# projectchrono/DEM-Engine

Hardware: AMD Instinct MI355X
Metric: clump*steps/s (higher is better)
Workload: dtype f32 physics / f64 geometry

## Files before the change

### dem-engine_amd/abi.py

```python
import ctypes as C
import os

import numpy as np

_HERE = os.path.dirname(os.path.abspath(__file__))

NULL_MAPPING_PARTNER = 0xFFFFFFFF
FAMILY_MASK_ENTRIES = 32896
NUM_FAMILIES = 256
FAMILY_FIXED = 1
FAMILY_GHOST = 2
FAMILY_PRESCRIBED = 4
INTEGRATOR_FORWARD_EULER, INTEGRATOR_CENTERED_DIFFERENCE, INTEGRATOR_EXTENDED_TAYLOR = 0, 1, 2
FORCE_HERTZIAN, FORCE_HERTZIAN_FRICTIONLESS, FORCE_CUSTOM = 0, 1, 2
GHOST_BYTES = 56


ARITH_FAST, ARITH_EXACT = 1, 0


class DemeParams(C.Structure):
    _fields_ = [
        ("nvXp2", C.c_uint32), ("nvYp2", C.c_uint32), ("nvZp2", C.c_uint32),
        ("nbX", C.c_uint32), ("nbY", C.c_uint32), ("nbZ", C.c_uint32),
# ... 145 lines not shown
        "deme_integrate": [_P], "deme_step": [_P, C.c_uint32],
        "deme_get_counts": [_P, C.POINTER(DemeCounts)],
        "deme_download_bin_incidence": [_P, _P, _P, C.c_size_t],
        "deme_download_contacts": [_P, _P, _P, _P, _P, C.c_size_t],
        "deme_download_contact_wildcard": [_P, C.c_uint32, _P, C.c_size_t],
        "deme_upload_contact_wildcard": [_P, C.c_uint32, _P, C.c_size_t],
        "deme_seed_contacts": [_P, _P, _P, _P, _P, C.c_size_t],
        "deme_compile_prescriptions": [_P, C.c_char_p, C.c_char_p, C.c_char_p],
        "deme_upload_wildcard_array": [_P, C.c_uint32, C.c_uint32, _P, C.c_size_t],
        "deme_download_wildcard_array": [_P, C.c_uint32, C.c_uint32, _P, C.c_size_t],
        "deme_halo_stream": [_P, C.POINTER(_P)], "deme_halo_pack_async": [_P, _P, C.c_uint32, _P],
        "deme_halo_unpack_async": [_P, _P, C.c_uint32, _P], "deme_halo_sync": [_P],
        "deme_step_overlap_begin": [_P, C.POINTER(C.c_int)], "deme_step_overlap_end": [_P],
        "deme_compile_family_rules": [_P, C.c_char_p], "deme_change_family": [_P, C.c_uint32, C.c_uint32],
        "deme_set_family_material": [_P, C.c_uint32, C.c_uint32, C.c_int],
        "deme_device_memory": [_P, C.POINTER(C.c_size_t), C.POINTER(C.c_size_t)],
        "deme_set_adaptive": [_P, C.POINTER(DemeAdaptive)],
        "deme_get_adaptive_state": [_P, C.POINTER(C.c_double), C.POINTER(C.c_uint32), C.POINTER(C.c_uint32), C.POINTER(C.c_uint32)],
        "deme_mark_persistent_contacts": [_P, C.c_int, C.c_uint32, C.c_uint32, C.c_int],
        "deme_num_persistent_contacts": [_P, C.POINTER(C.c_size_t)],
        "deme_add_owner_acc": [_P, C.c_uint32, C.c_uint32, _P, _P],
        "deme_download_persistent_contacts": [_P, _P, _P, _P, C.c_size_t],
        "deme_upload_persistent_contacts": [_P, _P, _P, _P, C.c_size_t],
        "deme_inspect": [_P, C.c_uint32, C.POINTER(C.c_float)],
        "deme_compile_region": [_P, C.c_char_p, C.POINTER(C.c_int)],
        "deme_inspect_region": [_P, C.c_uint32, C.c_int, C.POINTER(C.c_float)],
        "deme_upload_volumes": [_P, _P, C.c_size_t], "deme_inspect_values": [_P, C.c_uint32, _P, C.c_size_t],
        "deme_set_record_contacts": [_P, C.c_int],
        "deme_download_contact_records": [_P, _P, _P, _P, _P, C.c_size_t],
        "deme_download_sphere_geometry": [_P, _P, _P, _P, _P, C.c_size_t],
        "deme_query_owner_contacts": [_P, _P, C.c_size_t, C.c_int, _P, _P, _P, _P, _P, _P, _P, _P, _P, _P, C.c_size_t,
                                      C.POINTER(C.c_size_t)],
        "deme_query_host_bytes": [_P, C.POINTER(C.c_uint64)],
        "deme_change_owner_sizes": [_P, _P, _P, C.c_size_t], "deme_num_components": [_P, C.POINTER(C.c_uint32)],
        "deme_download_components": [_P, _P, _P, _P, _P, C.c_size_t], "deme_download_sphere_components": [_P, _P, C.c_size_t],
        "deme_set_template_components": [_P, C.c_uint32], "deme_multi_change_owner_sizes": [_P, _P, _P, C.c_size_t],
        "deme_multi_download_sphere_components": [_P, _P, C.c_size_t],
        "deme_compile_force_model": [_P, C.c_char_p, C.c_size_t, C.POINTER(C.c_char_p), C.c_uint32, C.c_char_p],
        "deme_compile_force_model_ex": [_P, C.c_char_p, C.c_size_t, C.POINTER(C.c_char_p), C.c_uint32, C.POINTER(C.c_char_p),
                                        C.c_uint32, C.POINTER(C.c_char_p), C.c_uint32, C.c_char_p],
        "deme_kernel_time_ms": [_P, C.c_char_p, C.POINTER(C.c_double), C.POINTER(C.c_uint64)],
        "deme_kernel_time_reset": [_P], "deme_set_timing": [_P, C.c_int],
        "deme_halo_pack": [_P, _P, C.c_uint32, _P], "deme_halo_unpack": [_P, _P, C.c_uint32, _P],
        "deme_jit_probe": [C.c_char_p, C.POINTER(C.c_char_p), C.c_uint32, C.c_char_p, C.c_char_p, C.c_size_t],
        "deme_jit_probe_ex": [C.c_char_p, C.POINTER(C.c_char_p), C.c_uint32, C.POINTER(C.c_char_p), C.c_uint32,
                              C.POINTER(C.c_char_p), C.c_uint32, C.c_char_p, C.c_char_p, C.c_size_t],
    }.items():
        fn = getattr(lib, name)
        fn.argtypes = args
        fn.restype = C.c_int
    lib.deme_halo_unique_id.argtypes = [_P]
    lib.deme_halo_unique_id.restype = C.c_int
    lib.deme_halo_group_create.argtypes = [_P, C.c_int, C.c_int, C.c_int, C.POINTER(_P)]
    lib.deme_halo_group_create.restype = C.c_int
    lib.deme_halo_group_destroy.argtypes = [_P]
    lib.deme_halo_group_destroy.restype = None
    lib.deme_halo_group_last_error.argtypes = [_P]
    lib.deme_halo_group_last_error.restype = C.c_char_p
    lib.deme_halo_group_attach.argtypes = [_P, _P, C.c_int, _P, _P, C.c_uint32, _P, C.c_uint32, C.c_int, _P, _P, C.c_uint32, _P, C.c_uint32]
    lib.deme_halo_group_attach.restype = C.c_int
    for name, args in {"deme_halo_group_step": [_P, C.c_uint32], "deme_halo_group_exchange": [_P], "deme_halo_group_sync": [_P],
                       "deme_halo_group_stats": [_P, C.POINTER(C.c_uint64), C.POINTER(C.c_uint64)]}.items():
        getattr(lib, name).argtypes = args
        getattr(lib, name).restype = C.c_int
    _lib = lib
    return lib


def halo_unique_id():
    buf = (C.c_ubyte * 128)()
    if load_library().deme_halo_unique_id(buf) != 0:
        raise DemeError("RCCL is not available (deme_halo_unique_id)")
    return bytes(buf)


class HaloGroup:

    def __init__(self, rank=0, world=1, device=0, unique_id=None):
        self.lib = load_library()
        h = _P()
        idbuf = None if unique_id is None else (C.c_ubyte * 128).from_buffer_copy(unique_id)
        rc = self.lib.deme_halo_group_create(idbuf, int(rank), int(world), int(device), C.byref(h))
        self.h = h
# ... 358 lines not shown
        self._ck(self.lib.deme_multi_download_contact_wildcard(self.h, int(w), _ptr(out), n), "deme_multi_download_contact_wildcard")
        return out

    def contact_records(self):
        n = self.num_contacts()
        arrs = [np.zeros((n, 3), np.float32) for _ in range(4)]
        self.lib.deme_multi_download_contact_records.argtypes = [_P, _P, _P, _P, _P, C.c_size_t]
        self._ck(self.lib.deme_multi_download_contact_records(self.h, *[_ptr(a) for a in arrs], n), "deme_multi_download_contact_records")
        return arrs

    def close(self):
        if getattr(self, "h", None):
            self.lib.deme_multi_destroy(self.h)
            self.h = None

    def __del__(self):
        try:
            self.close()
        except Exception:
            pass


def exported_symbols():
    import re
    hdr = os.path.join(_HERE, "..", "include", "deme_hip.h")
    txt = open(hdr).read()
    return sorted(set(re.findall(r"\b(deme_[a-z_0-9]+)\s*\(", txt)))


def _ptr(a):
    return None if a is None else a.ctypes.data


def jit_probe(src, wildcard_names=(), prerequisites="", owner_wildcards=(), geo_wildcards=()):
    lib = load_library()

    def arr(ns):
        return (C.c_char_p * max(1, len(ns)))(*[s.encode() for s in ns])
    log = C.create_string_buffer(8192)
    rc = lib.deme_jit_probe_ex(src.encode(), arr(wildcard_names), len(wildcard_names), arr(owner_wildcards), len(owner_wildcards),
                               arr(geo_wildcards), len(geo_wildcards), prerequisites.encode(), log, len(log))
    return rc == 0, log.value.decode(errors="replace")


class Context:

    def __init__(self, device=0):
        self.lib = load_library()
        h = _P()
        rc = self.lib.deme_ctx_create(int(device), C.byref(h))
        if rc != 0 or not h:
            raise DemeError(f"deme_ctx_create failed (status {rc}): is a HIP device visible?")
        self.h = h
        self.n_owners = 0
        self.n_spheres = 0
        self.n_wildcards = 0

    @classmethod
    def borrowed(cls, handle):
        self = cls.__new__(cls)
        self.lib = load_library()
        self.h = handle
        self._borrowed = True
        v = (C.c_uint32 * 4)()
        self.lib.deme_scene_sizes.argtypes = [_P, C.POINTER(C.c_uint32)]
        self._ck(self.lib.deme_scene_sizes(self.h, v), "deme_scene_sizes")
# ... 377 lines not shown
```

### dem-engine_amd/csrc/deme_hip.hip

```cpp
#include <algorithm>
#include <cmath>
#include <cstdarg>
#include <cstdio>
#include <cstdlib>
#include <chrono>
#include <cstring>
#include <condition_variable>
#include <functional>
#include <memory>
#include <mutex>
#include <dlfcn.h>
#include <map>
#include <string>
#include <thread>
#include <vector>

#include <hip/hip_runtime.h>
#include <rocprim/rocprim.hpp>
template <unsigned RB, unsigned IPT = 8>
using DemeRadixCfg = rocprim::radix_sort_config<rocprim::default_config, rocprim::default_config,
                                                rocprim::radix_sort_onesweep_config<rocprim::kernel_config<1024, IPT>, rocprim::kernel_config<1024, IPT>, RB,
                                                                                    rocprim::block_radix_rank_algorithm::match>,
                                                1024 * 1024>;
#include <array>
#include <iterator>
#include <limits>

#include "../../include/deme_hip.h"
#include "deme_device.h"
#include "deme_force.h"
#include "deme_force_fast.h"
#include "deme_jit.h"
#include "deme_kernels.h"
#include "deme_tile.h"
#include "deme_tile_step.h"
#include "deme_migrate.h"
#include "deme_mesh_kernels.h"
#include "deme_resize.h"
#include "deme_query.h"

using namespace deme_dev;

namespace {

struct DevBuf {
    void* p = nullptr;
    size_t bytes = 0;
    template <typename T>
    T* as() const {
        return reinterpret_cast<T*>(p);
    }
};

struct ContactList {
    DevBuf mapping, ownerA, ownerB[2], bIdx[2], info, tInfo, rIdx, lPos, remVal, rankC, remKey[2], cDefer, blockMode, smFlag, smList;
    DevBuf aStart, bStart, heavy, fixedFlag, heavyList, rangeCtr, hList, hCount, tileMode, tileOrg, rStart, lOff, lCount, tileRem, tileBase,
        tileBig, bigList;
    uint64_t nListed = 0;
    int listKeys = 0;
    bool legacyLists = false;
    bool tileActive = false;
    bool fusedList = false;
    bool fusedChecked = false;
    bool hrPending = false, heavyOverflow = false;
    uint32_t nHeavy = 0, nHeavyFree = 0, nSA = 0, nSM = 0;
    uint32_t nBigTiles = 0, tileMaxHalo = 0, tileMaxList = 0, tileMaxHaloIn = 0;

    void invalidate() {
        nListed = 0, listKeys = 0;
        legacyLists = tileActive = fusedList = fusedChecked = hrPending = heavyOverflow = false;
        nHeavy = nHeavyFree = nSA = nSM = 0;
        nBigTiles = tileMaxHalo = tileMaxList = tileMaxHaloIn = 0;
// ... 193 lines not shown
        HIPCK(hipMemcpyAsync(np, b.p, b.bytes, hipMemcpyDeviceToDevice, c->stream));
    if (b.p) {
        HIPCK(hipStreamSynchronize(c->stream));
        HIPCK(hipFree(b.p));
    }
    b.p = np;
    b.bytes = want;
    return DEME_OK;
}

template <typename T>
int upload(deme_ctx* c, DevBuf& b, const T* src, size_t n) {
    int rc = ensure(c, b, std::max<size_t>(n, 1) * sizeof(T));
    if (rc)
        return rc;
    if (n && src)
        HIPCK(hipMemcpyAsync(b.p, src, n * sizeof(T), hipMemcpyHostToDevice, c->stream));
    else if (n)
        HIPCK(hipMemsetAsync(b.p, 0, n * sizeof(T), c->stream));
    return DEME_OK;
}

template <class Call>
int with_temp(deme_ctx* c, DevBuf& tmp, Call&& call) {
    size_t bytes = 0;
    HIPCK(call(nullptr, bytes));
    if (int rc = ensure(c, tmp, bytes))
        return rc;
    bytes = tmp.bytes;
    HIPCK(call(tmp.p, bytes));
    return DEME_OK;
}

inline unsigned grid_for(size_t n, unsigned block = 256) { return (unsigned)((n + block - 1) / block); }
inline unsigned bits_for(uint64_t n, unsigned cap) {
    unsigned b = 1;
    while (b < cap && (1ull << b) < n)
        b++;
    return b;
}

hipEvent_t get_event(deme_ctx* c) {
    if (!c->eventPool.empty()) {
        hipEvent_t e = c->eventPool.back();
        c->eventPool.pop_back();
        return e;
    }
    hipEvent_t e;
    hipEventCreate(&e);
    return e;
}
struct ScopedTimer {
    deme_ctx* c;
    TimerSlot* slot = nullptr;
    hipEvent_t a = nullptr, b = nullptr;
    hipStream_t st = nullptr;
    ScopedTimer(deme_ctx* ctx, const char* name, bool always = false, hipStream_t stream = nullptr) : c(ctx), st(stream ? stream : ctx->stream) {
        if (!c->timing)
            return;
        slot = &c->timers[name];
        if (!always && (slot->seen++ % (uint64_t)c->timing) != 0) {
            slot = nullptr;
            return;
        }
        if (slot->pending.size() >= 8192) {
            slot = nullptr;
// ... 235 lines not shown
                return fail(c, DEME_ERR_OVERFLOW,
                            "a sphere touches more than %u bins (margin far larger than the bin size): the incidence list cannot be built",
                            DEME_MAX_BINS_PER_SPHERE);
            if ((uint64_t)hc.maxCount * nS > 0xFFFFFFFFull) {
                auto in64 = rocprim::make_transform_iterator(c->counts.as<uint32_t>(),
                                                             [] __host__ __device__(uint32_t v) { return (unsigned long long)v; });
                unsigned long long* tot = &c->ctr.as<DetectCounters>()->nContactsRaw;
                unsigned long long keep = 0, total = 0;
                HIPCK(hipMemcpyAsync(&keep, tot, 8, hipMemcpyDeviceToHost, st));
                if (int rc = with_temp(c, c->sortTmp, [&](void* tmp, size_t& bytes) {
                        return rocprim::reduce(tmp, bytes, in64, tot, 0ull, (size_t)nS, rocprim::plus<unsigned long long>(), st);
                    }))
                    return rc;
                HIPCK(hipMemcpyAsync(&total, tot, 8, hipMemcpyDeviceToHost, st));
                HIPCK(hipStreamSynchronize(st));
                HIPCK(hipMemcpyAsync(tot, &keep, 8, hipMemcpyHostToDevice, st));
                HIPCK(hipStreamSynchronize(st));
                if (total > 0xFFFFFFFFull)
                    return fail(c, DEME_ERR_OVERFLOW, "%llu bin-sphere incidences do not fit the 32-bit list offsets (use larger bins)", total);
            }
        }
        if (P > c->incCap) {
            if (int rc = grow_incidence_arena(c, (size_t)P + P / 4 + 1024))
                return rc;
            filled = false;
        }
        c->nInc = P;
        const unsigned bits = bits_for((uint64_t)c->hp.nbX * c->hp.nbY * c->hp.nbZ, 32);
        if (P) {
            if (!filled)
                fill_incidence();
            const bool twoPass = bits > 16 && bits <= 22;
            if (int rc = with_temp(c, c->sortTmp, [&](void* tmp, size_t& bytes) {
                    return twoPass ? rocprim::radix_sort_pairs<DemeRadixCfg<11, 16>>(tmp, bytes, c->incKeys[0].as<uint32_t>(), c->incKeys[1].as<uint32_t>(),
                                                                                     c->incVals[0].as<uint32_t>(), c->incVals[1].as<uint32_t>(), (size_t)P, 0, bits, st)
                                   : rocprim::radix_sort_pairs<DemeRadixCfg<8>>(tmp, bytes, c->incKeys[0].as<uint32_t>(), c->incKeys[1].as<uint32_t>(),
                                                                                c->incVals[0].as<uint32_t>(), c->incVals[1].as<uint32_t>(), (size_t)P, 0, bits, st);
                }))
                return rc;
            const uint32_t nWin = (uint32_t)grid_for(P, SW_T);
            if (int rc = ensure(c, c->binStat, (size_t)nWin * sizeof(uint2)))
                return rc;
            static_assert(SW_WPB == 1, "k_sweep writes one statistics record per window");
            hipLaunchKernelGGL(k_sweep, dim3(nWin), dim3(SW_T), 0, st, c->dp,
                               c->incKeys[1].as<uint32_t>(), c->incVals[1].as<uint32_t>(), P, c->geo.as<GeoRec>(),
                               c->sphFam.as<uint16_t>(), ar, c->binStat.as<uint2>());
            hipLaunchKernelGGL(k_bin_stats_final, dim3((nWin + 2047u) / 2048u), dim3(256), 0, st, c->binStat.as<uint2>(), nWin,
                               c->ctr.as<DetectCounters>());
        }
        c->nTriInc = 0;
        if (c->nTri && P) {
            const uint32_t nT = c->nTri;
            hipLaunchKernelGGL(k_tri_prep, dim3(grid_for(nT)), dim3(256), 0, st, c->dp, nT, c->tris.as<TriRec>(),
                               ow, c->triWorld.as<TriWorld>(), c->triLo.as<int4>(),
                               c->triHi.as<int4>(), c->triCounts.as<uint32_t>());
            size_t tmp = c->scanTmp.bytes;
            HIPCK(rocprim::exclusive_scan(c->scanTmp.p, tmp, c->triCounts.as<uint32_t>(), c->triOffsets.as<uint32_t>(), 0u,
                                          (size_t)nT + 1, rocprim::plus<uint32_t>(), st));
            uint32_t TP = 0;
            HIPCK(hipMemcpyAsync(&TP, c->triOffsets.as<uint32_t>() + nT, 4, hipMemcpyDeviceToHost, st));
            HIPCK(hipStreamSynchronize(st));
            if (TP > c->triCap) {
                const size_t cap = (size_t)TP + TP / 4 + 1024;
                for (int k = 0; k < 2; k++)
                    if (ensure(c, c->triKeys[k], cap * 4) || ensure(c, c->triVals[k], cap * 4))
                        return c->lastStatus;
                c->triCap = cap;
            }
            c->nTriInc = TP;
            if (TP) {
// ... 53 lines not shown
                        "a bin contains %u sphere components, exceeding the allowance %u (SetMaxSphereInBin)", c->maxInBin,
                        c->dp.errOutBinSphNum);
        uint64_t nC = hc.nContactsRaw;
        const size_t nPersist = c->hPersist.size();
        if (nPersist) {
            if (nC + nPersist > c->cntCap) {
                if (async)
                HIPCK(hipStreamSynchronize(c->stream));
            if (int rc = grow_contact_arena(c, (size_t)nC + nPersist + nC / 4 + 1024))
                    return rc;
                continue;
            }
            nC += nPersist;
        }
        const int next = c->keysCur ^ 1;
        uint64_t* rawKeys = c->keysRaw.as<uint64_t>();
        if (segmented) {
            c->lastSegMax = segMax;
            if (grid_for(segMax) > compactBlocks)
                hipLaunchKernelGGL(k_compact_keys, dim3((unsigned)grid_for(segMax) - compactBlocks, DEME_KEY_SEGS), dim3(256), 0, st,
                                   c->keysRaw.as<uint64_t>(), ar.segCap, c->segCtr.as<unsigned long long>(), compactBlocks,
                                   c->keysSorted[next].as<uint64_t>());
            if (hc.nContactsRaw)
                rawKeys = c->keysSorted[next].as<uint64_t>();
        }
        if (nPersist)
            HIPCK(hipMemcpyAsync(rawKeys + hc.nContactsRaw, c->persistKeys.p, nPersist * 8, hipMemcpyDeviceToDevice, st));
        if (nC) {
            const unsigned bitsA = bits_for(c->dp.nSpheres, 31);
            if (int rc = ensure(c, c->keysMid, (size_t)c->cntCap * 8))
                return rc;
            uint64_t* mid = c->keysMid.as<uint64_t>();
            if (int rc = with_temp(c, c->sortTmp, [&](void* tmp, size_t& bytes) {
                    return rocprim::radix_sort_keys<DemeRadixCfg<8>>(tmp, bytes, rawKeys, mid, (size_t)nC, 31, 33 + bitsA, st);
                }))
                return rc;
            hipLaunchKernelGGL(k_segment_rank_sort, dim3(grid_for(nC)), dim3(256), 0, st, (uint32_t)nC, mid,
                               c->keysSorted[next].as<uint64_t>());
            if (nPersist) {
                unsigned long long* cnt = &c->ctr.as<DetectCounters>()->nContactsRaw;
                if (int rc = with_temp(c, c->scanTmp, [&](void* tmp, size_t& bytes) {
                        return rocprim::unique(tmp, bytes, c->keysSorted[next].as<uint64_t>(), c->keysRaw.as<uint64_t>(), cnt, (size_t)nC,
                                               rocprim::equal_to<uint64_t>(), st);
                    }))
                    return rc;
                unsigned long long nU = 0;
                HIPCK(hipMemcpyAsync(&nU, cnt, 8, hipMemcpyDeviceToHost, st));
                HIPCK(hipStreamSynchronize(st));
                nC = nU;
                HIPCK(hipMemcpyAsync(c->keysSorted[next].p, c->keysRaw.p, (size_t)nC * 8, hipMemcpyDeviceToDevice, st));
            }
        }
        *nCout = nC;
        return DEME_OK;
    }
    return fail(c, DEME_ERR_OVERFLOW, "contact arena kept overflowing");
}

int build_legacy_lists(deme_ctx* c, ContactList& L, const OwnerRec* ow, hipStream_t st) {
    const uint64_t nC = L.nListed;
    if (nC) {
        const unsigned obits = bits_for(c->nOwners, 32);
        if (int rc = with_temp(c, c->sortTmp, [&](void* tmp, size_t& bytes) {
                return rocprim::radix_sort_pairs(tmp, bytes, L.ownerB[0].as<uint32_t>(), L.ownerB[1].as<uint32_t>(), L.bIdx[0].as<uint32_t>(),
                                                 L.bIdx[1].as<uint32_t>(), (size_t)nC, 0, obits, st);
            }))
            return rc;
// ... 80 lines not shown
        hipLaunchKernelGGL(k_run_starts, dim3(grid_for(nC)), dim3(256), 0, st, (uint32_t)nC, L.ownerA.as<uint32_t>(), c->nOwners,
                           L.aStart.as<uint32_t>());
    } else {
        HIPCK(hipMemsetAsync(L.aStart.p, 0, ((size_t)c->nOwners + 1) * 4, st));
    }
    L.nListed = nC, L.listKeys = next;
    bool tiled = false;
    RangeCounters hr{};
    if (tileEligible) {
        if (int rc = with_temp(c, c->scanTmp, [&](void* tmp, size_t& bytes) {
                return rocprim::exclusive_scan(tmp, bytes, L.tileRem.as<uint32_t>(), L.tileBase.as<uint32_t>(), 0u, (size_t)nTiles + 1,
                                               rocprim::plus<uint32_t>(), st);
            }))
            return rc;
        hipLaunchKernelGGL(k_tile_build, dim3(nTiles), dim3(256), 0, st, c->dp, c->nOwners, L.info.as<uint4>(),
                           L.ownerB[0].as<uint32_t>(), L.aStart.as<uint32_t>(), ow, L.tileBase.as<uint32_t>(), L.tInfo.as<uint2>(),
                           L.hList.as<uint32_t>(), L.hCount.as<uint32_t>(),
                           c->hasGhosts ? L.tileMode.as<uint32_t>() : (uint32_t*)nullptr, L.lOff.as<uint16_t>(),
                           L.lPos.as<uint16_t>(), L.lCount.as<uint32_t>(), L.rankC.as<uint32_t>(), L.remKey[0].as<uint32_t>(),
                           L.remVal.as<uint32_t>(), L.tileOrg.as<int64_t>(), L.rangeCtr.as<RangeCounters>(), nTiles,
                           L.tileBig.as<uint32_t>(), L.bigList.as<uint32_t>(), c->recContact.as<uint32_t>());
        hipLaunchKernelGGL(k_tile_stats, dim3((nTiles + 1023u) / 1024u), dim3(256), 0, st, nTiles, L.hCount.as<uint32_t>(),
                           L.lCount.as<uint32_t>(), L.rangeCtr.as<RangeCounters>());
        uint32_t nR = 0;
        HIPCK(hipMemcpyAsync(pin_at<uint32_t>(c, 8), L.tileBase.as<uint32_t>() + nTiles, 4, hipMemcpyDeviceToHost, st));
        HIPCK(hipMemcpyAsync(pin_at<RangeCounters>(c, 128), L.rangeCtr.p, sizeof(hr), hipMemcpyDeviceToHost, st));
        HIPCK(sync_readback(c, st, true));
        nR = *pin_at<uint32_t>(c, 8), hr = *pin_at<RangeCounters>(c, 128);
        nR += hr.nExtra;
        L.nBigTiles = hr.nBig;
        const unsigned obits = bits_for(c->nOwners, 32);
        if (nR) {
            if (int rc = with_temp(c, c->sortTmp, [&](void* tmp, size_t& bytes) {
                    return rocprim::radix_sort_pairs<DemeRadixCfg<10>>(tmp, bytes, L.remKey[0].as<uint32_t>(), L.remKey[1].as<uint32_t>(),
                                                                       L.remVal.as<uint32_t>(), L.rIdx.as<uint32_t>(), (size_t)nR, 0, obits, st);
                }))
                return rc;
            hipLaunchKernelGGL(k_run_starts, dim3(grid_for(nR)), dim3(256), 0, st, nR, L.remKey[1].as<uint32_t>(), c->nOwners,
                               L.rStart.as<uint32_t>());
        } else {
            HIPCK(hipMemsetAsync(L.rStart.p, 0, ((size_t)c->nOwners + 1) * 4, st));
        }
        hipLaunchKernelGGL(k_owner_ranges_tile, dim3(grid_for(c->nOwners)), dim3(256), 0, st, c->dp, ow, L.aStart.as<uint32_t>(),
                           L.lOff.as<uint16_t>(), L.rStart.as<uint32_t>(), L.heavy.as<uint8_t>(), L.fixedFlag.as<uint8_t>(),
                           L.heavyList.as<uint32_t>(), (uint32_t)(L.heavyList.bytes / 4), L.rangeCtr.as<RangeCounters>());
        tiled = true;
        static const int fusedEnv = getenv("DEME_FUSED") ? atoi(getenv("DEME_FUSED")) : -1;
        const int fusedMode = fusedEnv < 0 ? c->fusedEnable : fusedEnv;
        if ((fusedMode == 2 ? c->nOwners <= DEME_FUSED_AUTO_MAX_OWNERS : fusedMode != 0) && hr.nBig == 0 && c->hp.forceModel != DEME_FORCE_CUSTOM && !c->record && c->nTri == 0 &&
            !c->hasGhosts && !c->prescFn && !c->rulesFn && c->hShared.empty() && c->asyncLead == 0 &&
            !c->ad.autoBinSize && !c->ad.autoUpdateFreq) {
            hipLaunchKernelGGL(k_in_count, dim3(grid_for((size_t)c->nOwners + 1)), dim3(256), 0, st, c->dp, ow,
                               L.rStart.as<uint32_t>(), c->inCnt.as<uint32_t>());
            if (int rc = with_temp(c, c->scanTmp, [&](void* tmp, size_t& bytes) {
                    return rocprim::exclusive_scan(tmp, bytes, c->inCnt.as<uint32_t>(), c->inStart.as<uint32_t>(), 0u, (size_t)c->nOwners + 1,
                                                   rocprim::plus<uint32_t>(), st);
                }))
                return rc;
            hipLaunchKernelGGL(k_tile_incoming, dim3(nTiles), dim3(256), 0, st, c->dp, c->nOwners, L.info.as<uint4>(),
                               L.rStart.as<uint32_t>(), L.rIdx.as<uint32_t>(), c->recContact.as<uint32_t>(), c->inStart.as<uint32_t>(),
                               L.hList.as<uint32_t>(), L.hCount.as<uint32_t>(), c->hCountIn.as<uint32_t>(), c->tInfoIn.as<uint2>(),
                               c->inContact.as<uint32_t>(), L.rangeCtr.as<RangeCounters>());
            L.fusedList = true;
        }
    }
    if (tiled) {
        if (!c->hrPinned) {
            HIPCK(hipHostMalloc((void**)&c->hrPinned, sizeof(RangeCounters), hipHostMallocDefault));
// ... 3364 lines not shown
    for (uint32_t i = 0; i < nHit; i++) {
        const QueryHit& q = h[perm[i]];
        const uint32_t cls = key_class(q.key);
        if (idA)
            idA[i] = key_a(q.key);
        if (idB)
            idB[i] = key_b(q.key);
        if (type)
            type[i] = cls == DEME_KEY_CLASS_SS   ? DEME_SPHERE_SPHERE_CONTACT
                      : cls == DEME_KEY_CLASS_SM ? DEME_SPHERE_MESH_CONTACT
                      : c->hObjType[key_b(q.key)] == DEME_ANAL_OBJ_TYPE_PLANE ? DEME_SPHERE_PLANE_CONTACT
                                                                              : DEME_SPHERE_CYL_CONTACT;
        if (ownerA)
            ownerA[i] = q.ownerA;
        if (ownerB)
            ownerB[i] = q.ownerB;
        if (side)
            side[i] = (uint8_t)q.side;
        if (withRecords)
            for (int k = 0; k < 4; k++)
                if (dst[k])
                    memcpy(dst[k] + 3 * (size_t)i, r.data() + 12 * (size_t)perm[i] + 3 * k, 12);
    }
    return DEME_OK;
}

int deme_query_host_bytes(const deme_ctx* c, uint64_t* bytes) {
    if (!c || !bytes)
        return DEME_ERR_INVALID;
    *bytes = c->qHostBytes;
    return DEME_OK;
}

#include "deme_decomp.inc"
```

### include/deme_hip.h

```cpp
#ifndef DEME_HIP_H
#define DEME_HIP_H

#include <stddef.h>
#include <stdint.h>

#ifdef __cplusplus
extern "C" {
#endif

#define DEME_NOT_A_CONTACT 0
#define DEME_SPHERE_SPHERE_CONTACT 1
#define DEME_SPHERE_MESH_CONTACT 2
#define DEME_SPHERE_PLANE_CONTACT 11
#define DEME_SPHERE_CYL_CONTACT 13

#define DEME_ANAL_OBJ_TYPE_PLANE 0
#define DEME_ANAL_OBJ_TYPE_PLATE 1
#define DEME_ANAL_OBJ_TYPE_CYL_INF 2

#define DEME_NULL_MAPPING_PARTNER 0xFFFFFFFFu
#define DEME_NULL_BINID 0xFFFFFFFFu
#define DEME_NUM_FAMILIES 256
#define DEME_FAMILY_MASK_ENTRIES 32896
#define DEME_MAX_WILDCARD_NUM 16
// ... 121 lines not shown
int deme_order_probe(const DemeParams* p, size_t nClumps, const uint64_t* voxelID, const uint16_t* locX, const uint16_t* locY,
                     const uint16_t* locZ, uint32_t* order, double spread[2]);

int deme_set_params(deme_ctx* ctx, const DemeParams* p);
int deme_upload_scene(deme_ctx* ctx, const DemeScene* s);
int deme_upload_owner_state(deme_ctx* ctx, const DemeOwnerState* st);
int deme_download_owner_state(deme_ctx* ctx, DemeOwnerState* st);
int deme_update_tri_nodes(deme_ctx* ctx, const float* n1, const float* n2, const float* n3);

int deme_compute_margins(deme_ctx* ctx, uint32_t drift);
int deme_set_margins(deme_ctx* ctx, const float* marginSize);

int deme_detect_contacts(deme_ctx* ctx);
int deme_migrate_history(deme_ctx* ctx);
int deme_calc_forces(deme_ctx* ctx);
int deme_integrate(deme_ctx* ctx);
int deme_step(deme_ctx* ctx, uint32_t nsteps);
int deme_set_async_detection(deme_ctx* ctx, uint32_t leadSteps);

int deme_get_counts(deme_ctx* ctx, DemeCounts* out);

int deme_download_bin_incidence(deme_ctx* ctx, uint32_t* binIDs, uint32_t* sphereIDs, size_t cap);
int deme_download_contacts(deme_ctx* ctx, uint32_t* idA, uint32_t* idB, uint8_t* type, uint32_t* mapping, size_t cap);
int deme_download_contact_wildcard(deme_ctx* ctx, uint32_t w, float* out, size_t cap);
int deme_upload_contact_wildcard(deme_ctx* ctx, uint32_t w, const float* in, size_t n);
int deme_seed_contacts(deme_ctx* ctx, const uint32_t* idA, const uint32_t* idB, const uint8_t* type, const float* wildcards,
                       size_t n);
int deme_set_record_contacts(deme_ctx* ctx, int enable);
int deme_download_contact_records(deme_ctx* ctx, float* force, float* torqueOnly, float* cpA, float* cpB, size_t cap);
int deme_query_owner_contacts(deme_ctx* ctx, const uint32_t* ownerIds, size_t nOwners, int withRecords, uint32_t* idA, uint32_t* idB,
                              uint8_t* type, uint32_t* ownerA, uint32_t* ownerB, uint8_t* side, float* force, float* torqueOnly,
                              float* cpA, float* cpB, size_t cap, size_t* nOut);
int deme_query_host_bytes(const deme_ctx* ctx, uint64_t* bytes);
int deme_download_sphere_geometry(deme_ctx* ctx, double* X, double* Y, double* Z, float* R, size_t cap);

int deme_change_owner_sizes(deme_ctx* ctx, const uint32_t* ownerIds, const float* factors, size_t n);
int deme_num_components(const deme_ctx* ctx, uint32_t* n);
int deme_download_components(deme_ctx* ctx, float* relX, float* relY, float* relZ, float* radius, size_t cap);
int deme_download_sphere_components(deme_ctx* ctx, uint16_t* comp, size_t cap);
int deme_set_template_components(deme_ctx* ctx, uint32_t n);

int deme_compile_force_model(deme_ctx* ctx, const char* src, size_t len, const char* const* wildcardNames,
                             uint32_t nWildcards, const char* prerequisites);

int deme_compile_prescriptions(deme_ctx* ctx, const char* velCases, const char* posCases, const char* accCases);

int deme_compile_family_rules(deme_ctx* ctx, const char* rules);
int deme_change_family(deme_ctx* ctx, uint32_t from, uint32_t to);

typedef struct DemeAdaptive {
    uint32_t autoBinSize;
    uint32_t binObserveSteps;
    float binMaxRate;
    float binAcc;
    float binUpperSafety;
    float binLowerSafety;
    uint32_t autoUpdateFreq;
    uint32_t maxUpdateFreq;
    uint32_t freqObserveDetections;
} DemeAdaptive;
int deme_set_adaptive(deme_ctx* ctx, const DemeAdaptive* a);
int deme_get_adaptive_state(deme_ctx* ctx, double* binSize, uint32_t* cdUpdateFreq, uint32_t* nBinChanges, uint32_t* nFreqChanges);

int deme_add_owner_acc(deme_ctx* ctx, uint32_t owner, uint32_t n, const float* acc, const float* angAcc);

int deme_mark_persistent_contacts(deme_ctx* ctx, int mode, uint32_t N1, uint32_t N2, int mark);
// ... 135 lines not shown
```

Baseline: 6.314 billion.

## Add custom LSD radix sort and use it for large contact-detection sorts

Introduces a hand-written three-kernel-per-pass LSD radix sort (count, row scan, wave-ballot ranked scatter through shared memory) and routes the bin-incidence, 64-bit contact-key and removal-record sorts to it once element counts pass per-site thresholds, with rocPRIM kept for smaller inputs. The aim is to cut the cost of rocPRIM onesweep sorts on large inputs in the detection pipeline. It also exports host-facing test entry points for the sort. In exchange it needs extra scratch space for a ping-pong buffer and a tile table, and uses three launches per 8-bit pass, which may be slower than onesweep for some sizes or bit widths.

```diff
diff --git a/dem-engine_amd/abi.py b/dem-engine_amd/abi.py
--- a/dem-engine_amd/abi.py
+++ b/dem-engine_amd/abi.py
@@ -201,6 +201,8 @@
         "deme_query_owner_contacts": [_P, _P, C.c_size_t, C.c_int, _P, _P, _P, _P, _P, _P, _P, _P, _P, _P, C.c_size_t,
                                       C.POINTER(C.c_size_t)],
         "deme_query_host_bytes": [_P, C.POINTER(C.c_uint64)],
+        "deme_sort_pairs_u32": [C.c_int, _P, _P, C.c_size_t, C.c_uint, C.c_uint, C.c_int, _P, _P],
+        "deme_sort_keys_u64": [C.c_int, _P, C.c_size_t, C.c_uint, C.c_uint, C.c_int, _P],
         "deme_change_owner_sizes": [_P, _P, _P, C.c_size_t], "deme_num_components": [_P, C.POINTER(C.c_uint32)],
         "deme_download_components": [_P, _P, _P, _P, _P, C.c_size_t], "deme_download_sphere_components": [_P, _P, C.c_size_t],
         "deme_set_template_components": [_P, C.c_uint32], "deme_multi_change_owner_sizes": [_P, _P, _P, C.c_size_t],
@@ -218,6 +220,8 @@
         fn = getattr(lib, name)
         fn.argtypes = args
         fn.restype = C.c_int
+    lib.deme_sort_tile_keys.argtypes = []
+    lib.deme_sort_tile_keys.restype = C.c_uint
     lib.deme_halo_unique_id.argtypes = [_P]
     lib.deme_halo_unique_id.restype = C.c_int
     lib.deme_halo_group_create.argtypes = [_P, C.c_int, C.c_int, C.c_int, C.POINTER(_P)]
@@ -642,6 +646,31 @@
     return None if a is None else a.ctypes.data
 
 
+def sort_tile_keys():
+    return int(load_library().deme_sort_tile_keys())
+
+
+def sort_pairs_u32(keys, vals, begin_bit, end_bit, force_own=True, device=0):
+    keys, vals = np.ascontiguousarray(keys, np.uint32), np.ascontiguousarray(vals, np.uint32)
+    assert keys.shape == vals.shape and keys.ndim == 1
+    ko, vo = np.empty_like(keys), np.empty_like(vals)
+    rc = load_library().deme_sort_pairs_u32(device, _ptr(keys), _ptr(vals), keys.size, begin_bit, end_bit, int(bool(force_own)), _ptr(ko),
+                                            _ptr(vo))
+    if rc:
+        raise DemeError(f"deme_sort_pairs_u32 failed with code {rc}")
+    return ko, vo
+
+
+def sort_keys_u64(keys, begin_bit, end_bit, force_own=True, device=0):
+    keys = np.ascontiguousarray(keys, np.uint64)
+    assert keys.ndim == 1
+    ko = np.empty_like(keys)
+    rc = load_library().deme_sort_keys_u64(device, _ptr(keys), keys.size, begin_bit, end_bit, int(bool(force_own)), _ptr(ko))
+    if rc:
+        raise DemeError(f"deme_sort_keys_u64 failed with code {rc}")
+    return ko
+
+
 def jit_probe(src, wildcard_names=(), prerequisites="", owner_wildcards=(), geo_wildcards=()):
     lib = load_library()
 
diff --git a/dem-engine_amd/csrc/deme_hip.hip b/dem-engine_amd/csrc/deme_hip.hip
--- a/dem-engine_amd/csrc/deme_hip.hip
+++ b/dem-engine_amd/csrc/deme_hip.hip
@@ -38,6 +38,7 @@
 #include "deme_mesh_kernels.h"
 #include "deme_resize.h"
 #include "deme_query.h"
+#include "deme_sort.h"
 
 using namespace deme_dev;
 
@@ -297,6 +298,26 @@
     return DEME_OK;
 }
 
+#ifndef DEME_SORT_ROCPRIM
+#define DEME_SORT_ROCPRIM 0
+#endif
+constexpr size_t DEME_SORT_OWN_FROM_INCIDENCES = 82000;
+constexpr size_t DEME_SORT_OWN_FROM_KEYS64 = 430000;
+constexpr size_t DEME_SORT_OWN_FROM_RECORDS = 180000;
+inline bool sort_takes_own(size_t n, size_t cap, size_t ownFrom) {
+    return !DEME_SORT_ROCPRIM && n >= ownFrom && std::max(n, cap) <= deme_sort::MAX_N;
+}
+template <class RocCfg, bool HAS_V, typename K>
+hipError_t deme_radix_sort(void* tmp, size_t& bytes, const K* keysIn, K* keysOut, const uint32_t* valsIn, uint32_t* valsOut, size_t n, size_t cap,
+                           unsigned beginBit, unsigned endBit, size_t ownFrom, hipStream_t st) {
+    if (sort_takes_own(n, cap, ownFrom))
+        return deme_sort::radix_sort<K, HAS_V>(tmp, bytes, keysIn, keysOut, valsIn, valsOut, n, cap, beginBit, endBit, st);
+    if constexpr (HAS_V)
+        return rocprim::radix_sort_pairs<RocCfg>(tmp, bytes, keysIn, keysOut, valsIn, valsOut, n, beginBit, endBit, st);
+    else
+        return rocprim::radix_sort_keys<RocCfg>(tmp, bytes, keysIn, keysOut, n, beginBit, endBit, st);
+}
+
 inline unsigned grid_for(size_t n, unsigned block = 256) { return (unsigned)((n + block - 1) / block); }
 inline unsigned bits_for(uint64_t n, unsigned cap) {
     unsigned b = 1;
@@ -598,10 +619,12 @@
                 fill_incidence();
             const bool twoPass = bits > 16 && bits <= 22;
             if (int rc = with_temp(c, c->sortTmp, [&](void* tmp, size_t& bytes) {
-                    return twoPass ? rocprim::radix_sort_pairs<DemeRadixCfg<11, 16>>(tmp, bytes, c->incKeys[0].as<uint32_t>(), c->incKeys[1].as<uint32_t>(),
-                                                                                     c->incVals[0].as<uint32_t>(), c->incVals[1].as<uint32_t>(), (size_t)P, 0, bits, st)
-                                   : rocprim::radix_sort_pairs<DemeRadixCfg<8>>(tmp, bytes, c->incKeys[0].as<uint32_t>(), c->incKeys[1].as<uint32_t>(),
-                                                                                c->incVals[0].as<uint32_t>(), c->incVals[1].as<uint32_t>(), (size_t)P, 0, bits, st);
+                    return twoPass ? deme_radix_sort<DemeRadixCfg<11, 16>, true>(tmp, bytes, c->incKeys[0].as<uint32_t>(), c->incKeys[1].as<uint32_t>(),
+                                                                                 c->incVals[0].as<uint32_t>(), c->incVals[1].as<uint32_t>(), (size_t)P,
+                                                                                 (size_t)c->incCap, 0, bits, DEME_SORT_OWN_FROM_INCIDENCES, st)
+                                   : deme_radix_sort<DemeRadixCfg<8>, true>(tmp, bytes, c->incKeys[0].as<uint32_t>(), c->incKeys[1].as<uint32_t>(),
+                                                                            c->incVals[0].as<uint32_t>(), c->incVals[1].as<uint32_t>(), (size_t)P,
+                                                                            (size_t)c->incCap, 0, bits, DEME_SORT_OWN_FROM_INCIDENCES, st);
                 }))
                 return rc;
             const uint32_t nWin = (uint32_t)grid_for(P, SW_T);
@@ -721,7 +744,8 @@
                 return rc;
             uint64_t* mid = c->keysMid.as<uint64_t>();
             if (int rc = with_temp(c, c->sortTmp, [&](void* tmp, size_t& bytes) {
-                    return rocprim::radix_sort_keys<DemeRadixCfg<8>>(tmp, bytes, rawKeys, mid, (size_t)nC, 31, 33 + bitsA, st);
+                    return deme_radix_sort<DemeRadixCfg<8>, false>(tmp, bytes, rawKeys, mid, nullptr, nullptr, (size_t)nC, (size_t)c->cntCap, 31,
+                                                                   33 + bitsA, DEME_SORT_OWN_FROM_KEYS64, st);
                 }))
                 return rc;
             hipLaunchKernelGGL(k_segment_rank_sort, dim3(grid_for(nC)), dim3(256), 0, st, (uint32_t)nC, mid,
@@ -868,8 +892,9 @@
         const unsigned obits = bits_for(c->nOwners, 32);
         if (nR) {
             if (int rc = with_temp(c, c->sortTmp, [&](void* tmp, size_t& bytes) {
-                    return rocprim::radix_sort_pairs<DemeRadixCfg<10>>(tmp, bytes, L.remKey[0].as<uint32_t>(), L.remKey[1].as<uint32_t>(),
-                                                                       L.remVal.as<uint32_t>(), L.rIdx.as<uint32_t>(), (size_t)nR, 0, obits, st);
+                    return deme_radix_sort<DemeRadixCfg<10>, true>(tmp, bytes, L.remKey[0].as<uint32_t>(), L.remKey[1].as<uint32_t>(),
+                                                                   L.remVal.as<uint32_t>(), L.rIdx.as<uint32_t>(), (size_t)nR, (size_t)c->cntCap, 0, obits,
+                                                                   DEME_SORT_OWN_FROM_RECORDS, st);
                 }))
                 return rc;
             hipLaunchKernelGGL(k_run_starts, dim3(grid_for(nR)), dim3(256), 0, st, nR, L.remKey[1].as<uint32_t>(), c->nOwners,
@@ -4300,4 +4325,74 @@
     return DEME_OK;
 }
 
+namespace {
+struct SortScratch {
+    std::vector<void*> held;
+    ~SortScratch() {
+        for (void* p : held)
+            (void)hipFree(p);
+    }
+    template <typename T>
+    T* room(size_t n) {
+        void* p = nullptr;
+        if (hipMalloc(&p, std::max<size_t>(n, 1) * sizeof(T)) != hipSuccess)
+            return nullptr;
+        held.push_back(p);
+        return reinterpret_cast<T*>(p);
+    }
+};
+template <class RocCfg, bool HAS_V, typename K>
+int sort_host_arrays(int device, const K* keys, const uint32_t* vals, size_t n, unsigned beginBit, unsigned endBit, size_t ownFrom, K* keysOut,
+                     uint32_t* valsOut) {
+    if (endBit < beginBit || endBit > 8 * sizeof(K) || (n && (!keys || !keysOut || (HAS_V && (!vals || !valsOut)))))
+        return DEME_ERR_INVALID;
+    if (!ownFrom && (DEME_SORT_ROCPRIM || n > deme_sort::MAX_N))
+        return DEME_ERR_INVALID;
+    if (!n)
+        return DEME_OK;
+    if (hipSetDevice(device) != hipSuccess)
+        return DEME_ERR_HIP;
+    SortScratch s;
+    K *dIn = s.room<K>(n), *dOut = s.room<K>(n);
+    uint32_t *vIn = HAS_V ? s.room<uint32_t>(n) : nullptr, *vOut = HAS_V ? s.room<uint32_t>(n) : nullptr;
+    if (!dIn || !dOut || (HAS_V && (!vIn || !vOut)))
+        return DEME_ERR_HIP;
+    size_t bytes = 0;
+    if (deme_radix_sort<RocCfg, HAS_V>(nullptr, bytes, dIn, dOut, vIn, vOut, n, n, beginBit, endBit, ownFrom, nullptr) != hipSuccess)
+        return DEME_ERR_HIP;
+    void* tmp = s.room<char>(bytes);
+    if (!tmp)
+        return DEME_ERR_HIP;
+    bool ok = hipMemcpy(dIn, keys, n * sizeof(K), hipMemcpyHostToDevice) == hipSuccess;
+    if (HAS_V)
+        ok = ok && hipMemcpy(vIn, vals, n * 4, hipMemcpyHostToDevice) == hipSuccess;
+    ok = ok && deme_radix_sort<RocCfg, HAS_V>(tmp, bytes, dIn, dOut, vIn, vOut, n, n, beginBit, endBit, ownFrom, nullptr) == hipSuccess;
+    ok = ok && hipDeviceSynchronize() == hipSuccess;
+    ok = ok && hipMemcpy(keysOut, dOut, n * sizeof(K), hipMemcpyDeviceToHost) == hipSuccess;
+    if (HAS_V)
+        ok = ok && hipMemcpy(valsOut, vOut, n * 4, hipMemcpyDeviceToHost) == hipSuccess;
+    return ok ? DEME_OK : DEME_ERR_HIP;
+}
+}
+
+unsigned deme_sort_tile_keys(void) { return deme_sort::TILE; }
+
+int deme_sort_pairs_u32(int device, const uint32_t* keys, const uint32_t* vals, size_t n, unsigned beginBit, unsigned endBit, int forceOwn,
+                        uint32_t* keysOut, uint32_t* valsOut) {
+    const unsigned bits = endBit >= beginBit ? endBit - beginBit : 0;
+    if (bits <= 20)
+        return sort_host_arrays<DemeRadixCfg<10>, true>(device, keys, vals, n, beginBit, endBit, forceOwn ? 0 : DEME_SORT_OWN_FROM_RECORDS, keysOut,
+                                                        valsOut);
+    if (bits <= 22)
+        return sort_host_arrays<DemeRadixCfg<11, 16>, true>(device, keys, vals, n, beginBit, endBit, forceOwn ? 0 : DEME_SORT_OWN_FROM_INCIDENCES,
+                                                            keysOut, valsOut);
+    return sort_host_arrays<DemeRadixCfg<8>, true>(device, keys, vals, n, beginBit, endBit, forceOwn ? 0 : DEME_SORT_OWN_FROM_INCIDENCES, keysOut,
+                                                   valsOut);
+}
+
+int deme_sort_keys_u64(int device, const uint64_t* keys, size_t n, unsigned beginBit, unsigned endBit, int forceOwn, uint64_t* keysOut) {
+    return sort_host_arrays<DemeRadixCfg<8>, false>(device, keys, nullptr, n, beginBit, endBit, forceOwn ? 0 : DEME_SORT_OWN_FROM_KEYS64, keysOut,
+                                                    nullptr);
+}
+
 #include "deme_decomp.inc"
diff --git a/dem-engine_amd/csrc/deme_sort.h b/dem-engine_amd/csrc/deme_sort.h
--- /dev/null
+++ b/dem-engine_amd/csrc/deme_sort.h
@@ -0,0 +1,206 @@
+#pragma once
+#include <cstdint>
+#include <hip/hip_runtime.h>
+#include <rocprim/block/block_scan.hpp>
+
+namespace deme_sort {
+
+#ifndef DEME_SORT_THREADS
+#define DEME_SORT_THREADS 512
+#endif
+#ifndef DEME_SORT_KPT
+#define DEME_SORT_KPT 8
+#endif
+constexpr unsigned THREADS = DEME_SORT_THREADS, WAVE = 64, WAVES = THREADS / WAVE;
+constexpr unsigned SCAN_THREADS = 256;
+constexpr unsigned RB = 8, RADIX = 1u << RB;
+constexpr unsigned KPT = DEME_SORT_KPT;
+constexpr unsigned TILE = THREADS * KPT;
+constexpr unsigned SCAN_IPT = 16;
+constexpr size_t MAX_N = (size_t)1 << 31;
+static_assert(THREADS >= RADIX && THREADS % WAVE == 0, "one thread per digit in the histogram steps");
+static_assert(WAVE == 64, "ballots are 64 lanes wide");
+
+using BlockScan = rocprim::block_scan<uint32_t, THREADS>;
+using RowScan = rocprim::block_scan<uint32_t, SCAN_THREADS>;
+
+template <typename K>
+__device__ inline unsigned digit_of(K k, unsigned shift, unsigned mask) {
+    return (unsigned)(k >> shift) & mask;
+}
+
+template <typename K>
+__global__ __launch_bounds__(THREADS) void k_count(const K* __restrict__ keys, uint32_t n, uint32_t nTiles, unsigned shift, unsigned nbits,
+                                                   uint32_t* __restrict__ table) {
+    __shared__ uint32_t hist[RADIX];
+    const unsigned tid = threadIdx.x, tile = blockIdx.x, mask = (1u << nbits) - 1u;
+    if (tid < RADIX)
+        hist[tid] = 0;
+    __syncthreads();
+    const uint32_t base = tile * TILE + tid;
+#pragma unroll
+    for (unsigned i = 0; i < KPT; i++) {
+        const uint32_t idx = base + i * THREADS;
+        if (idx < n)
+            atomicAdd(&hist[digit_of(keys[idx], shift, mask)], 1u);
+    }
+    __syncthreads();
+    if (tid <= mask)
+        table[(size_t)tid * nTiles + tile] = hist[tid];
+}
+
+__global__ __launch_bounds__(SCAN_THREADS) void k_scan_rows(uint32_t* __restrict__ table, uint32_t nTiles, uint32_t* __restrict__ totals) {
+    __shared__ typename RowScan::storage_type scanSt;
+    uint32_t* row = table + (size_t)blockIdx.x * nTiles;
+    uint32_t carry = 0;
+    for (uint32_t base = 0; base < nTiles; base += SCAN_THREADS * SCAN_IPT) {
+        const uint32_t first = base + threadIdx.x * SCAN_IPT;
+        uint32_t v[SCAN_IPT], sum = 0;
+#pragma unroll
+        for (unsigned i = 0; i < SCAN_IPT; i++) {
+            v[i] = first + i < nTiles ? row[first + i] : 0u;
+            sum += v[i];
+        }
+        uint32_t excl, total;
+        RowScan().exclusive_scan(sum, excl, 0u, total, scanSt);
+        __syncthreads();
+        uint32_t run = carry + excl;
+#pragma unroll
+        for (unsigned i = 0; i < SCAN_IPT; i++) {
+            if (first + i < nTiles)
+                row[first + i] = run;
+            run += v[i];
+        }
+        carry += total;
+    }
+    if (threadIdx.x == 0)
+        totals[blockIdx.x] = carry;
+}
+
+template <typename K, bool HAS_V>
+__global__ __launch_bounds__(THREADS) void k_scatter(const K* __restrict__ keys, const uint32_t* __restrict__ vals, uint32_t n, uint32_t nTiles,
+                                                     unsigned shift, unsigned nbits, const uint32_t* __restrict__ table,
+                                                     const uint32_t* __restrict__ totals, K* __restrict__ keysOut, uint32_t* __restrict__ valsOut) {
+    __shared__ typename BlockScan::storage_type scanSt;
+    __shared__ K sKeys[TILE];
+    __shared__ uint32_t sVals[HAS_V ? TILE : 1];
+    __shared__ uint32_t wcnt[WAVES * RADIX];
+    __shared__ uint32_t gbase[RADIX];
+    const unsigned tid = threadIdx.x, lane = tid % WAVE, w = tid / WAVE, tile = blockIdx.x, mask = (1u << nbits) - 1u;
+    const uint32_t tile0 = tile * TILE, nValid = n - tile0 < TILE ? n - tile0 : TILE;
+    for (unsigned d = tid; d < WAVES * RADIX; d += THREADS)
+        wcnt[d] = 0;
+    K k[KPT];
+    uint32_t v[KPT], rank[KPT];
+#pragma unroll
+    for (unsigned i = 0; i < KPT; i++) {
+        const uint32_t at = w * (WAVE * KPT) + i * WAVE + lane;
+        k[i] = at < nValid ? keys[tile0 + at] : ~K(0);
+        if (HAS_V)
+            v[i] = at < nValid ? vals[tile0 + at] : 0u;
+    }
+    __syncthreads();
+    uint32_t* wc = wcnt + w * RADIX;
+#pragma unroll
+    for (unsigned i = 0; i < KPT; i++) {
+        const unsigned d = digit_of(k[i], shift, mask);
+        unsigned long long same = ~0ull;
+#pragma unroll
+        for (unsigned b = 0; b < RB; b++) {
+            const bool bit = (d >> b) & 1u;
+            const unsigned long long bal = __ballot(bit);
+            same &= bit ? bal : ~bal;
+        }
+        const uint32_t before = __hip_atomic_load(wc + d, __ATOMIC_RELAXED, __HIP_MEMORY_SCOPE_WAVEFRONT);
+        if ((same >> lane) == 1ull)
+            __hip_atomic_fetch_add(wc + d, (uint32_t)__popcll(same), __ATOMIC_RELAXED, __HIP_MEMORY_SCOPE_WAVEFRONT);
+        rank[i] = before + (uint32_t)__popcll(same & ((1ull << lane) - 1ull));
+    }
+    __syncthreads();
+    const unsigned dt = tid % RADIX;
+    uint32_t pre[WAVES], c = 0;
+#pragma unroll
+    for (unsigned j = 0; j < WAVES; j++) {
+        pre[j] = c;
+        c += tid < RADIX ? wcnt[j * RADIX + dt] : 0u;
+    }
+    uint32_t dstart, dbase;
+    BlockScan().exclusive_scan(c, dstart, 0u, scanSt);
+    __syncthreads();
+    BlockScan().exclusive_scan(tid <= mask ? totals[tid] : 0u, dbase, 0u, scanSt);
+    if (tid < RADIX) {
+#pragma unroll
+        for (unsigned j = 0; j < WAVES; j++)
+            wcnt[j * RADIX + dt] = dstart + pre[j];
+    }
+    if (tid <= mask)
+        gbase[tid] = dbase + table[(size_t)tid * nTiles + tile] - dstart;
+    __syncthreads();
+#pragma unroll
+    for (unsigned i = 0; i < KPT; i++) {
+        const uint32_t p = wcnt[w * RADIX + digit_of(k[i], shift, mask)] + rank[i];
+        sKeys[p] = k[i];
+        if (HAS_V)
+            sVals[p] = v[i];
+    }
+    __syncthreads();
+#pragma unroll
+    for (unsigned i = 0; i < KPT; i++) {
+        const uint32_t p = i * THREADS + tid;
+        if (p < nValid) {
+            const K key = sKeys[p];
+            const uint32_t o = gbase[digit_of(key, shift, mask)] + p;
+            if (o < n) {
+                keysOut[o] = key;
+                if (HAS_V)
+                    valsOut[o] = sVals[p];
+            }
+        }
+    }
+}
+
+inline size_t align256(size_t b) { return (b + 255) & ~(size_t)255; }
+inline unsigned passes_for(unsigned beginBit, unsigned endBit) { return (endBit - beginBit + RB - 1) / RB; }
+
+template <typename K, bool HAS_V>
+hipError_t radix_sort(void* tmp, size_t& bytes, const K* keysIn, K* keysOut, const uint32_t* valsIn, uint32_t* valsOut, size_t n, size_t cap,
+                      unsigned beginBit, unsigned endBit, hipStream_t st) {
+    const size_t room = n > cap ? n : cap, tilesRoom = (room + TILE - 1) / TILE;
+    const size_t tableB = align256((tilesRoom + 1) * RADIX * 4), keysB = align256(room * sizeof(K)), valsB = HAS_V ? align256(room * 4) : 0;
+    if (!tmp) {
+        bytes = tableB + keysB + valsB;
+        return hipSuccess;
+    }
+    if (bytes < tableB + keysB + valsB || room > MAX_N || endBit < beginBit || endBit > 8 * sizeof(K))
+        return hipErrorInvalidValue;
+    if (!n)
+        return hipSuccess;
+    const unsigned passes = passes_for(beginBit, endBit);
+    if (!passes) {
+        hipError_t e = hipMemcpyAsync(keysOut, keysIn, n * sizeof(K), hipMemcpyDeviceToDevice, st);
+        if (e == hipSuccess && HAS_V)
+            e = hipMemcpyAsync(valsOut, valsIn, n * 4, hipMemcpyDeviceToDevice, st);
+        return e;
+    }
+    uint32_t* table = reinterpret_cast<uint32_t*>(tmp);
+    uint32_t* totals = table + tilesRoom * RADIX;
+    K* keysAlt = reinterpret_cast<K*>(reinterpret_cast<char*>(tmp) + tableB);
+    uint32_t* valsAlt = reinterpret_cast<uint32_t*>(reinterpret_cast<char*>(tmp) + tableB + keysB);
+    const uint32_t nTiles = (uint32_t)((n + TILE - 1) / TILE);
+    const K* kSrc = keysIn;
+    const uint32_t* vSrc = valsIn;
+    for (unsigned p = 0; p < passes; p++) {
+        const unsigned shift = beginBit + p * RB, nbits = endBit - shift < RB ? endBit - shift : RB;
+        const bool toOut = (passes - 1 - p) % 2 == 0;
+        K* kDst = toOut ? keysOut : keysAlt;
+        uint32_t* vDst = toOut ? valsOut : valsAlt;
+        hipLaunchKernelGGL(k_count<K>, dim3(nTiles), dim3(THREADS), 0, st, kSrc, (uint32_t)n, nTiles, shift, nbits, table);
+        hipLaunchKernelGGL(k_scan_rows, dim3(1u << nbits), dim3(SCAN_THREADS), 0, st, table, nTiles, totals);
+        hipLaunchKernelGGL((k_scatter<K, HAS_V>), dim3(nTiles), dim3(THREADS), 0, st, kSrc, vSrc, (uint32_t)n, nTiles, shift, nbits, table,
+                           totals, kDst, vDst);
+        kSrc = kDst, vSrc = vDst;
+    }
+    return hipGetLastError();
+}
+
+}
diff --git a/include/deme_hip.h b/include/deme_hip.h
--- a/include/deme_hip.h
+++ b/include/deme_hip.h
@@ -177,6 +177,10 @@
                               uint8_t* type, uint32_t* ownerA, uint32_t* ownerB, uint8_t* side, float* force, float* torqueOnly,
                               float* cpA, float* cpB, size_t cap, size_t* nOut);
 int deme_query_host_bytes(const deme_ctx* ctx, uint64_t* bytes);
+int deme_sort_pairs_u32(int device, const uint32_t* keys, const uint32_t* vals, size_t n, unsigned beginBit, unsigned endBit, int forceOwn,
+                        uint32_t* keysOut, uint32_t* valsOut);
+int deme_sort_keys_u64(int device, const uint64_t* keys, size_t n, unsigned beginBit, unsigned endBit, int forceOwn, uint64_t* keysOut);
+unsigned deme_sort_tile_keys(void);
 int deme_download_sphere_geometry(deme_ctx* ctx, double* X, double* Y, double* Z, float* R, size_t cap);
 
 int deme_change_owner_sizes(deme_ctx* ctx, const uint32_t* ownerIds, const float* factors, size_t n);
```

Result: faster. 6.389 billion (median of 6 runs) (+1.2%).
